# DallinClark/RealTimeRaytracer

Hardware: AMD Instinct MI355X
Metric: Mrays/sec at 1920x1080 1spp (all rays: primary + shadow) (higher is better)
Workload: dtype f32

## Files before the change

realtimeraytracer_amd/csrc/kernels/rtr_device.h:

```cpp
#pragma once
#include <hip/hip_runtime.h>
#include <stdint.h>
#include "../../../include/rtr_types.h"
#include "../../../include/rtr_math.h"

namespace rtrdev {

struct DeviceTexture { const uint8_t* pixels; uint32_t width, height, channels, _pad; };

constexpr uint32_t kLightTriRecord = 4;

struct DeviceScene {
    const uint4* nodes;
    const RtrBvhGrid* grid;
    const uint4* nodes4;
    uint32_t numNodes4;
    const float4* tris;
    const RtrVertex* vertices;
    const uint32_t* indices;
    const RtrObjectInfo* objects;
    const RtrAreaLightInfo* lights;
    const float4* lightTris;
    const uint32_t* lightTriFirst;
    const float* xforms;
    const float* nmats;
    const float* ltc1;
    const float* ltc2;
    float skyLinear[3];
    uint32_t numLights;
    uint32_t numLightTris;
    const DeviceTexture* textures;
    DeviceTexture hdri;
};

struct Counters {
// ... 251 lines not shown
    if (LIMIT > 0 && over) { best.custom = RTR_STACK_OVERFLOW; best.prim = RTR_MISS; best.t = tmax; best.u = 0.f; best.v = 0.f; best.leaf = 0; return false; }
    return found;
}

#define RTR_PI_F 3.14159265359f
__device__ __forceinline__ float chiGGX(float v) { return v > 0.0f ? 1.0f : 0.0f; }
__device__ __forceinline__ float GGX_Distribution(rtr_v3 n, rtr_v3 h, float alpha) {
    const float NoH = rtr_dot(n, h);
    const float alpha2 = alpha * alpha;
    const float NoH2 = NoH * NoH;
    const float den = rtr_max(rtr_fma(NoH2, alpha2, 1.0f - NoH2), 0.001f);
    return (chiGGX(NoH) * alpha2) / (RTR_PI_F * den * den);
}
__device__ __forceinline__ float GGX_PartialGeometryTerm(rtr_v3 v, rtr_v3 n, rtr_v3 h, float alpha) {
    float VoH2 = rtr_clamp(rtr_dot(v, h), 0.001f, 1.0f);
    const float chi = chiGGX(VoH2 / rtr_clamp(rtr_dot(v, n), 0.001f, 1.0f));
    VoH2 = VoH2 * VoH2;
    const float tan2 = (1.0f - VoH2) / VoH2;
    return (chi * 2.0f) / (1.0f + rtr_sqrt(rtr_fma(alpha * alpha, tan2, 1.0f)));
}
__device__ __forceinline__ rtr_v3 Fresnel_Schlick(float cosT, rtr_v3 F0) {
    const float p = rtr_pow(1.0f - cosT, 5.0f);
    return rtr_mk(rtr_fma(1.0f - F0.x, p, F0.x), rtr_fma(1.0f - F0.y, p, F0.y), rtr_fma(1.0f - F0.z, p, F0.z));
}

#define RTR_LUT_SIZE 64.0f
#define RTR_LUT_SCALE ((RTR_LUT_SIZE - 1.0f) / RTR_LUT_SIZE)
#define RTR_LUT_BIAS (0.5f / RTR_LUT_SIZE)

__device__ __forceinline__ float4 sample_lut(const float* __restrict__ lut, float u, float v) {
    float x = rtr_fma(u, RTR_LUT_SIZE, -0.5f), y = rtr_fma(v, RTR_LUT_SIZE, -0.5f);
    if (!(x >= -1.0e6f && x <= 1.0e6f)) x = 0.0f;
    if (!(y >= -1.0e6f && y <= 1.0e6f)) y = 0.0f;
    const float x0f = __builtin_floorf(x), y0f = __builtin_floorf(y);
// ... 81 lines not shown
    return (size_t)(ra.directRows ? gy : lrow) * ra.width + px;
}

__device__ __forceinline__ rtr_v3 primary_dir(const RenderArgs& ra, uint32_t px, uint32_t py, uint32_t i) {
    const float jx = rtr_random(px + i), jy = rtr_random(px + i * 322u);
    const float offx = ((float)px + jx) - 0.5f, offy = ((float)py + jy) - 0.5f;
    const rtr_v3 pw = rtr_madd(rtr_madd(rtr_ld3(ra.cam.topLeftViewportCorner), rtr_ld3(ra.cam.horizontalViewportDelta), offx),
                               rtr_ld3(ra.cam.verticalViewportDelta), offy);
    return rtr_normalize(rtr_sub(pw, rtr_ld3(ra.cam.position)));
}

struct Accum { rtr_v3 analytic, shadowed, unshadowed, avgNormal, avgPosition; };

struct Surface {
    rtr_v3 hitPoint, hitNormal, viewDir, color, mDiffuse, mSpecular;
    float roughness, metallic, om;
    float4 t1, t2;
};

template <bool SHADE, bool STATS>
__device__ __forceinline__ bool fetch_surface(const DeviceScene& sc, const RenderArgs& ra, const HitRec& h, rtr_v3 rayDir,
                                              bool wantAnalytic, Accum& o, Surface& sf, LocalStats& st) {
    if (h.custom == RTR_MISS) {
        if (SHADE) {
            rtr_v3 sky = rtr_ld3(sc.skyLinear);
            if (sc.hdri.pixels) {
                const rtr_v3 dir = rtr_normalize(rayDir);
                const float hu = rtr_atan2(dir.z, dir.x) / (2.0f * 3.14159265f) + 0.5f;
                float hv = rtr_acos(rtr_clamp(dir.y, -1.0f, 1.0f)) / 3.14159265f;
                hv = 1.0f - hv;
                const float4 tx = sample_tex<STATS>(sc.hdri, hu, hv, st);
                sky = rtr_mk(rtr_to_linear(tx.x), rtr_to_linear(tx.y), rtr_to_linear(tx.z));
            }
// ... 24 lines not shown
    const rtr_v3 localPos = rtr_madd(rtr_madd(rtr_scale(p0, b0), p1, b1), p2, b2);
    const rtr_v3 hitPoint = rtr_xform_point34(sc.xforms + 12u * h.custom, localPos);
    const rtr_v3 nsum = rtr_madd(rtr_madd(rtr_scale(n0, b0), n1, b1), n2, b2);
    const float* nm = sc.nmats + 12u * h.custom;
    rtr_v3 hitNormal;
    if (rtr_dot(nsum, nsum) > 0.0f) {
        hitNormal = rtr_normalize(rtr_mul33(nm, rtr_normalize(nsum)));
    } else {
        const rtr_v3 g = rtr_cross(rtr_sub(p1, p0), rtr_sub(p2, p0));
        rtr_v3 n = rtr_normalize(rtr_mul33(nm, rtr_normalize(g)));
        if (rtr_dot(n, rayDir) > 0.0f) n = rtr_neg(n);
        hitNormal = n;
    }
    float metallic = oi->metallic;
    float rough = oi->specular;
    rtr_v3 color = rtr_mk(0, 0, 0);
    if (SHADE) {
        rtr_v3 col = rtr_ld3(oi->color);
        if (oi->usesColorMap | oi->usesSpecularMap | oi->usesMetallicMap) {
            const float4 ta = va[2], tb = vb[2], tc = vc[2];
            const float uu = rtr_fma(tc.x, b2, rtr_fma(tb.x, b1, ta.x * b0));
            const float vv = rtr_fma(tc.y, b2, rtr_fma(tb.y, b1, ta.y * b0));
            if (oi->usesColorMap != 0u) { const float4 t = sample_tex<STATS>(sc.textures[oi->colorIndex], uu, vv, st); col = rtr_mk(t.x, t.y, t.z); }
            if (oi->usesSpecularMap != 0u) rough = sample_tex<STATS>(sc.textures[oi->specularIndex], uu, vv, st).x;
            if (oi->usesMetallicMap != 0u) metallic = sample_tex<STATS>(sc.textures[oi->metallicIndex], uu, vv, st).x;
        }
        color = rtr_mk(rtr_to_linear(col.x), rtr_to_linear(col.y), rtr_to_linear(col.z));
    }
    const float roughness = 1.0f - rough;

    const rtr_v3 viewDir = rtr_normalize(rtr_sub(camPos, hitPoint));
    const float om = 1.0f - metallic;
    rtr_v3 mDiffuse = rtr_mk(0, 0, 0), mSpecular = rtr_mk(0, 0, 0);
    float4 t1 = make_float4(1, 0, 0, 1), t2 = make_float4(0, 0, 0, 0);
    if (SHADE) {
        o.avgNormal = rtr_add(o.avgNormal, hitNormal);
        o.avgPosition = rtr_add(o.avgPosition, hitPoint);
        mDiffuse = rtr_scale(color, om);
        mSpecular = rtr_mk(rtr_fma(color.x, metallic, 0.04f * om), rtr_fma(color.y, metallic, 0.04f * om),
                           rtr_fma(color.z, metallic, 0.04f * om));
        if (wantAnalytic) {
            const float dotNV = rtr_clamp(rtr_dot(hitNormal, viewDir), 0.0f, 1.0f);
            const float lu = rtr_fma(roughness, RTR_LUT_SCALE, RTR_LUT_BIAS);
            const float lv = rtr_fma(rtr_sqrt(1.0f - dotNV), RTR_LUT_SCALE, RTR_LUT_BIAS);
            t1 = sample_lut(sc.ltc1, lu, lv);
            t2 = sample_lut(sc.ltc2, lu, lv);
        }
    }
    sf.hitPoint = hitPoint; sf.hitNormal = hitNormal; sf.viewDir = viewDir; sf.color = color;
    sf.mDiffuse = mDiffuse; sf.mSpecular = mSpecular; sf.roughness = roughness; sf.metallic = metallic; sf.om = om;
    sf.t1 = t1; sf.t2 = t2;
    return true;
}

__device__ __forceinline__ rtr_v3 surface_diffuse(float om, rtr_v3 color) {
    return rtr_mk((om * color.x) / RTR_PI_F, (om * color.y) / RTR_PI_F, (om * color.z) / RTR_PI_F);
}
__device__ __forceinline__ rtr_v3 area_sample_contrib(rtr_v3 hitNormal, rtr_v3 viewDir, float roughness, rtr_v3 mSpecular, rtr_v3 currDiffuse,
                                                      rtr_v3 lcol, float lintensity, float pdf, rtr_v3 sampledLightDir, float lightDistance) {
    const rtr_v3 halfVector = rtr_normalize(rtr_add(viewDir, sampledLightDir));
    const float cosTheta = rtr_clamp(rtr_dot(viewDir, halfVector), 0.0f, 1.0f);
    const float Dg = GGX_Distribution(hitNormal, halfVector, roughness);
    const float G = GGX_PartialGeometryTerm(viewDir, hitNormal, halfVector, roughness) *
                    GGX_PartialGeometryTerm(sampledLightDir, hitNormal, halfVector, roughness);
    const rtr_v3 F = Fresnel_Schlick(cosTheta, mSpecular);
    const float NdotV = rtr_max(rtr_dot(hitNormal, viewDir), 0.1f);
    const float NdotL = rtr_max(rtr_dot(hitNormal, sampledLightDir), 0.1f);
    const float den = 4.0f * NdotV * NdotL;
    const rtr_v3 currSpecular = rtr_mk(((Dg * F.x) * G) / den, ((Dg * F.y) * G) / den, ((Dg * F.z) * G) / den);
    const float attenuation = 1.0f / (lightDistance * lightDistance);
    const rtr_v3 BRDF = rtr_add(currSpecular, currDiffuse);
    const rtr_v3 Lr = rtr_mk((((lcol.x * lintensity) * NdotL) * attenuation) * 10.0f, (((lcol.y * lintensity) * NdotL) * attenuation) * 10.0f,
// ... 34 lines not shown
    return light_sample_at(P, light_sample_pair(s + light_sample_seed0(px, py, frame)));
}
struct DrawnSamples {
    uint32_t px, py, frame;
    __device__ __forceinline__ SamplePair pair(uint32_t s) const { return light_sample_pair(s + light_sample_seed0(px, py, frame)); }
};

constexpr uint32_t kDirectionalSlot = 0xffffffffu;
#ifndef RTR_INTO_EXPR
#define RTR_INTO_EXPR (rtr_dot(hitNormal, lightVec) < 0.0f)
#endif
template <class Policy, bool STATS, class Samples>
__device__ __forceinline__ void light_loops_from(const DeviceScene& sc, const RenderArgs& ra, const Samples& smp,
                                                 const Surface& sf, uint32_t want, Accum& o, Policy& pol, LocalStats& st) {
    const bool wantAnalytic = (want & 1u) != 0u, wantUnshadowed = (want & 2u) != 0u;
    const rtr_v3 hitPoint = sf.hitPoint, hitNormal = sf.hitNormal, viewDir = sf.viewDir, color = sf.color;
    const rtr_v3 mDiffuse = sf.mDiffuse, mSpecular = sf.mSpecular;
    const float roughness = sf.roughness, om = sf.om;
    const float4 t1 = sf.t1, t2 = sf.t2;
    const rtr_v3 shadowOrigin = rtr_madd(hitPoint, hitNormal, 0.01f);
    const rtr_v3 currDiffuse = surface_diffuse(om, color);

    for (uint32_t li = 0; li < ra.info.numAreaLights; ++li) {
        const RtrAreaLightInfo* L = sc.lights + li;
        if (STATS) st.lightFetch++;
        const rtr_v3 lcol = rtr_ld3(L->color);
        const float lintensity = L->intensity;
        const uint32_t lnt = L->numTriangles;
        const bool twoSided = L->isTwoSided != 0u;
        for (uint32_t ti = 0; ti < lnt; ++ti) {
            if (STATS) st.lightTriFetch++;
            const float4* rec = sc.lightTris + (size_t)(sc.lightTriFirst[li] + ti) * kLightTriRecord;
            const float4 r0 = rec[0], r1 = rec[1], r2 = rec[2], r3 = rec[3];
            rtr_v3 P[3];
            P[0] = rtr_mk(r0.x, r0.y, r0.z); P[1] = rtr_mk(r1.x, r1.y, r1.z); P[2] = rtr_mk(r2.x, r2.y, r2.z);
            const float pdf = r1.w;
// ... 152 lines not shown
```

realtimeraytracer_amd/csrc/kernels/rtr_kernels.h:

```cpp
#pragma once
#include <hip/hip_runtime.h>
#include "rtr_device.h"

namespace rtrdev {

#ifndef RTR_SHADOW_FAR_FIRST
#define RTR_SHADOW_FAR_FIRST 1
#endif
#if RTR_SHADOW_FAR_FIRST
#define RTR_ANYHIT_KERNEL_REVISION "r05.3"
#else
#define RTR_ANYHIT_KERNEL_REVISION "r05.3-nearest-first"
#endif

constexpr uint32_t kQueueRegions = 8;
constexpr uint32_t kQueueLenWord = 0;
constexpr uint32_t kPrimaryRedoWord = 2;
constexpr uint32_t kOccludedWord = 3;
constexpr uint32_t kBatchCursorWord = 16;
static_assert(kOccludedWord < kBatchCursorWord && kPrimaryRedoWord < kOccludedWord, "the small counters sit below the first batch cursor");
constexpr uint32_t kQueueLists = kQueueRegions * kQueueRegions;
constexpr uint32_t kQueueListLens = kBatchCursorWord + 16 * kQueueLists;
constexpr uint32_t kPrimaryCursors = kQueueListLens + kQueueLists;
constexpr uint32_t kQueueCtrlWords = kPrimaryCursors + 16 * kQueueRegions;
// ... 71 lines not shown
    uint2* lists;
    uint32_t listStride;
    const int32_t* startLeaves;
    uint32_t numTris;
};
struct RayMaskArgs {
    const uint8_t* rayMasks = nullptr;
    uint32_t cullMask = 0xffu;
    uint32_t masked = 0;
};
hipError_t launch_occlusion_walk(const DeviceScene& sc, const OcclusionArgs& oa, const Tunables& tun, bool alpha, Counters* stats, hipStream_t stream, uint32_t numCus,
                                 const RayMaskArgs& rm = RayMaskArgs());

hipError_t launch_light_tris(const RtrAreaLightInfo* lights, const RtrVertex* vertices, const uint32_t* indices, const uint32_t* first,
                             uint32_t numLights, float4* out, hipStream_t stream);
hipError_t launch_deinterleave(const uint32_t* gathered, uint32_t* dst, uint32_t width, uint32_t height,
                               uint32_t bandRows, uint32_t shardCount, uint32_t localRows, hipStream_t stream);

}
```

realtimeraytracer_amd/csrc/kernels/rtr_kernels.hip:

```cpp
#include "rtr_kernels.h"

#include <algorithm>
#include <cstdlib>
#include <cstring>

namespace rtrdev {

constexpr int kBlock = 256;

template <bool STATS, int STACK>
struct InlinePolicy {
    static constexpr bool kShade = true;
    __device__ __forceinline__ void slots_at(uint32_t) {}
    const DeviceScene& sc; int32_t* stack; LocalStats& st;
    __device__ __forceinline__ bool occluded(rtr_v3 o, rtr_v3 d, float tmax, rtr_v3, bool) {
        HitRec h;
        return trace<true, STATS, kBlock>(sc, stack, o, d, 0.001f, tmax, h, st);
    }
};

__device__ __forceinline__ uint32_t wave_sum_u32(uint32_t v) {
#pragma unroll
    for (int o = 32; o > 0; o >>= 1) v += __shfl_xor(v, o);
    return v;
// ... 393 lines not shown
            }
        }
    }
}

constexpr size_t kBinnedMinRays = (size_t)10 << 20;
constexpr uint32_t kBinnedMinNodes = 1u << 16;
#ifndef RTR_GEN_OCT_BLOCK
#define RTR_GEN_OCT_BLOCK 512
#endif
constexpr uint32_t kGenOctBlock = RTR_GEN_OCT_BLOCK;
constexpr uint32_t kParkSurface = 6, kParkWords = kParkSurface + 2u * kParkedPairs;
#ifndef RTR_GEN_OCT_WAVES
#define RTR_GEN_OCT_WAVES 7
#endif
#if RTR_GEN_OCT_WAVES > 0
#define RTR_GEN_OCT_ATTR __attribute__((amdgpu_waves_per_eu(RTR_GEN_OCT_WAVES, 8)))
#else
#define RTR_GEN_OCT_ATTR
#endif
__global__ __launch_bounds__(kGenOctBlock) RTR_GEN_OCT_ATTR void k_shadow_gen_oct(DeviceScene sc, FrameBatch fb, const float4* hitTuvp, const uint32_t* hitCustom,
                                                              RayQueue queue, uint32_t* ctrl, uint32_t planeStride, uint2* lists,
                                                              uint32_t listStride, uint32_t kBatch, uint32_t nt) {
    constexpr uint32_t kWaves = kGenOctBlock / 64;
    __shared__ uint32_t s_tot[kWaves][8], s_run[kWaves][8];
    __shared__ uint32_t s_park[kParkWords * kGenOctBlock];
    uint32_t q;
    const uint32_t frame = batch_frame(blockIdx.x * kGenOctBlock + threadIdx.x, planeStride, q);
    const RenderArgs& ra = fb.ra[frame < fb.n ? frame : 0u];
    const size_t plane0 = (size_t)frame * ra.spp;
    const uint32_t wave = threadIdx.x >> 6;
    uint32_t px = 0, lrow = 0, py = 0;
    const bool live = frame < fb.n && pixel_of(ra, q, px, lrow, py);
    LocalStats st;
    Accum acc = zero_accum();
    const bool single = ra.spp == 1u;
    const lds_column park = (lds_column)&s_park[threadIdx.x];
    const ParkedSamples<kGenOctBlock> smp{park + kParkSurface * kGenOctBlock, light_sample_seed0(px, py, ra.info.frame), ra.numShadowRays <= kParkedPairs};
    CountOctPolicy cp{0ull, 0ull};
    if (live) {
        smp.draw(ra.numShadowRays);
        for (uint32_t i = 0; i < ra.spp; ++i) {
            const size_t k = (plane0 + i) * planeStride + q;
            const float4 r = hitTuvp[k];
            HitRec h; h.t = r.x; h.u = r.y; h.v = r.z; h.prim = __float_as_uint(r.w); h.custom = hitCustom[k];
            Surface sf;
            bool surf = fetch_surface<false, false>(sc, ra, h, primary_dir(ra, px, py, i), false, acc, sf, st);
#if RTR_EXP_DOUBLE_FETCH_GEN
            if (surf) {
                HitRec h2 = h; h2.u = h.u + sf.hitPoint.x * (float)(ra.spp - 1u) * 1.0e-30f; h2.v = h.v + sf.hitNormal.y * (float)(ra.spp - 1u) * 1.0e-30f;
                h2.prim = h.prim + (__float_as_uint(sf.hitPoint.z) == 0x7fc12345u ? 1u : 0u);
                Surface sf2;
                if (fetch_surface<false, false>(sc, ra, h2, primary_dir(ra, px, py, i), false, acc, sf2, st)) sf = sf2;
            }
#endif
            if (surf) {
                if (single) {
// ... 39 lines not shown
        uint32_t at = 0, pos = 0;
        if (threadIdx.x == 0 && total) at = atomicAdd(ctrl, total);
        if (cnt) pos = atomicAdd(ctrl + kQueueListLens + threadIdx.x, cnt);
        const uint32_t first = (uint32_t)__builtin_amdgcn_readfirstlane((int)at) + before;
        if (x == 0) {
            uint32_t c = first;
            for (uint32_t w = 0; w < kWaves; ++w) { s_run[w][o] = c; c += s_tot[w][o]; }
        }
        for (uint32_t j = 0; j < cnt; ++j) {
            const uint32_t f = (b0 + j * kQueueRegions) * kB;
            lists[(size_t)threadIdx.x * listStride + pos + j] = make_uint2(first + f, len - f < kB ? len - f : kB);
        }
    }
    __syncthreads();
    if (mine == 0) return;
    for (uint32_t i = 0; i < ra.spp; ++i) {
        const size_t k = (plane0 + i) * planeStride + q;
        EmitOctPolicy pol{queue, (EmitOctPolicy::lds_word)&s_run[wave][0], (uint32_t)k, nt};
        if (single) {
            Surface sf0 = {};
            sf0.hitPoint = rtr_mk(__uint_as_float(park[0u * kGenOctBlock]), __uint_as_float(park[1u * kGenOctBlock]), __uint_as_float(park[2u * kGenOctBlock]));
            sf0.hitNormal = rtr_mk(__uint_as_float(park[3u * kGenOctBlock]), __uint_as_float(park[4u * kGenOctBlock]), __uint_as_float(park[5u * kGenOctBlock]));
            queue_store_origin(queue, k, sf0.hitPoint, sf0.hitNormal);
            light_loops_from<EmitOctPolicy, false>(sc, ra, smp, sf0, 0u, acc, pol, st);
        } else {
            const float4 r = hitTuvp[k];
            HitRec h; h.t = r.x; h.u = r.y; h.v = r.z; h.prim = __float_as_uint(r.w); h.custom = hitCustom[k];
            Surface sf;
            if (fetch_surface<false, false>(sc, ra, h, primary_dir(ra, px, py, i), false, acc, sf, st)) {
                queue_store_origin(queue, k, sf.hitPoint, sf.hitNormal);
                light_loops_from<EmitOctPolicy, false>(sc, ra, smp, sf, 0u, acc, pol, st);
            }
        }
    }
// ... 882 lines not shown
        if (valid) {
            const float4 r = hitTuvp[k];
            HitRec h; h.t = r.x; h.u = r.y; h.v = r.z; h.prim = __float_as_uint(r.w); h.custom = hitCustom[k];
            has = fetch_surface<true, false>(sc, ra, h, primary_dir(ra, px, py, i), false, acc, sf, st);
#if RTR_EXP_DOUBLE_FETCH
            if (has) {
                HitRec h2 = h; h2.u = h.u + (float)(ra.spp - 1u) * 1.0e-30f; h2.v = h.v + (float)(ra.spp - 1u) * 1.0e-30f;
                Surface sf2; Accum acc2 = zero_accum();
                const bool has2 = fetch_surface<true, false>(sc, ra, h2, primary_dir(ra, px, py, i), false, acc2, sf2, st);
                if (has2 && sf2.roughness == 12345.0f && sf2.hitPoint.x == 4321.0f && sf2.color.y == 777.0f && sf2.viewDir.z == 55.0f && sf2.hitNormal.y == 99.0f) sf = sf2;
            }
#endif
        }
        wave_lds_sync();
        if (has) {
            const rtr_v3 cd = surface_diffuse(sf.om, sf.color);
            s_surf[wave][0][lane] = make_float4(sf.hitPoint.x, sf.hitPoint.y, sf.hitPoint.z, sf.roughness);
            s_surf[wave][1][lane] = make_float4(sf.hitNormal.x, sf.hitNormal.y, sf.hitNormal.z, cd.x);
            s_surf[wave][2][lane] = make_float4(sf.viewDir.x, sf.viewDir.y, sf.viewDir.z, cd.y);
            s_surf[wave][3][lane] = make_float4(sf.mSpecular.x, sf.mSpecular.y, sf.mSpecular.z, cd.z);
        }
        const rtr_v3 hitPoint = sf.hitPoint, hitNormal = sf.hitNormal;
        uint32_t qdone = 0;
        rtr_v3 shadowedSample = rtr_mk(0, 0, 0);
        uint32_t e0 = 0, total = 0;
        do {
            uint32_t count = 0, e = 0, e1 = e0;
            uint32_t vmask = 0, imask = 0;
            bool full = false;
            const uint32_t occ = has ? vis_mask32(vis, (uint32_t)k + qdone * slotStride, slotStride, ra.maxRaysPerSample - qdone) : 0xffffffffu;
            uint32_t nq = 0;
// ... 101 lines not shown
        const uint32_t band = y / bandRows, r = y % bandRows;
        const uint32_t shard = band % shardCount, lb = band / shardCount;
        dst[p] = gathered[((size_t)shard * localRows + (size_t)lb * bandRows + r) * width + x];
    }
}

__global__ __launch_bounds__(64) void k_light_tris(const RtrAreaLightInfo* __restrict__ lights, const RtrVertex* __restrict__ vertices,
                                                   const uint32_t* __restrict__ indices, const uint32_t* __restrict__ first,
                                                   uint32_t numLights, float4* __restrict__ out) {
    const uint32_t l = blockIdx.x * 64u + threadIdx.x;
    if (l >= numLights) return;
    const RtrAreaLightInfo* L = lights + l;
    for (uint32_t ti = 0; ti < L->numTriangles; ++ti) light_tri_record(L, vertices, indices, ti, out + (size_t)(first[l] + ti) * kLightTriRecord);
}

__global__ __launch_bounds__(kBlock) void k_fill_planes(uint4* __restrict__ vis, uint32_t word, uint32_t planeVec, uint32_t pitchVec,
                                                        uint32_t* __restrict__ ctrl, uint32_t ctrlWords, uint32_t* __restrict__ overflowCount) {
    if (blockIdx.x == 0 && blockIdx.y == 0) {
        for (uint32_t i = threadIdx.x; i < ctrlWords; i += kBlock) ctrl[i] = 0u;
        if (threadIdx.x == 0) overflowCount[0] = 0u;
    }
    const uint4 v = make_uint4(word, word, word, word);
    uint4* plane = vis + (size_t)blockIdx.y * pitchVec;
    for (uint32_t i = blockIdx.x * kBlock + threadIdx.x; i < planeVec; i += gridDim.x * kBlock) plane[i] = v;
}

namespace {
struct TunableField { const char* name; uint32_t Tunables::* field; uint32_t lo, hi; };
const TunableField kTunables[] = {
    {"primary_packet", &Tunables::primary_packet, 0u, 1u}, {"primary_wide", &Tunables::primary_wide, 0u, 1u}, {"primary_persist", &Tunables::primary_persist, 0u, 2u}, {"primary_persist_min_rays", &Tunables::primary_persist_min_rays, 0u, 0xffffffffu},
// ... 96 lines not shown
    }
    if (ev) hipEventRecord(ev[1], s);
    const uint32_t kBatchEnv = tun.trace_batch;
    const uint32_t kBatch = kBatchEnv >= 64u ? kBatchEnv : ((size_t)nb * blocks * kBlock * ra.spp * ra.maxRaysPerSample >= kBatchLongQueue ? kBatchLong : kBatchDefault);
    const uint32_t kWide = tun.trace_bvh4;
    const uint32_t genBlocks = (nb * blocks * kBlock + kGenBlock - 1) / kGenBlock, genOctBlocks = (nb * blocks * kBlock + kGenOctBlock - 1) / kGenOctBlock;
    const uint32_t binMode = tun.trace_binned;
    const size_t maxRaysQ = (size_t)nb * blocks * kBlock * ra.spp * ra.maxRaysPerSample;
    const bool wide = kWide && sc.nodes4;
    const bool binned = wide && ws.batchLists && (size_t)ra.spp * ra.maxRaysPerSample <= 65535u &&
                        (size_t)ws.capRays / kBatch / kQueueRegions + genOctBlocks <= ws.listStride &&
                        (binMode == 1u || (binMode == 2u && maxRaysQ >= kBinnedMinRays && sc.numNodes4 >= kBinnedMinNodes));
    const uint32_t kNtQueue = tun.queue_nt;
    RayQueue rq = ws.rayQueue;
    rq.ownLeaf = (wide && tun.trace_own_leaf) ? 1u : 0u;
    if (binned) hipLaunchKernelGGL(k_shadow_gen_oct, dim3(genOctBlocks), dim3(kGenOctBlock), 0, s, sc, fb, ws.hitTuvp, ws.hitCustom, rq, ws.queueCount, blocks * kBlock, ws.batchLists, ws.listStride, kBatch, kNtQueue >> 1);
    else hipLaunchKernelGGL(k_shadow_gen, dim3(genBlocks), dim3(kGenBlock), 0, s, sc, fb, ws.hitTuvp, ws.hitCustom, rq, ws.queueCount, blocks * kBlock);
    if (ev) hipEventRecord(ev[2], s);
    const size_t maxRays = (size_t)nb * blocks * kBlock * ra.spp * ra.maxRaysPerSample;
    const uint32_t kWgsPerCu = tun.trace_wgs_per_cu;
    uint32_t tblocks = numCus * (kWgsPerCu ? kWgsPerCu : (maxRays >= kBinnedMinRays ? 8u : 6u));
    const uint32_t needed = (uint32_t)((maxRays + kBlock - 1) / kBlock);
    if (tblocks > needed) tblocks = needed;
    if (tblocks == 0) tblocks = 1;
    const uint32_t kRefill = tun.trace_refill, kInnerMin = tun.trace_inner_min;
    (void)sizeof(STACK);
    const uint32_t kOct = tun.trace_octant_forms | ((kNtQueue & 1u) << 1);
    const uint32_t kTop = tun.trace_top_nodes < kTopNodes ? tun.trace_top_nodes : kTopNodes;
    const uint32_t top = kTop < sc.numNodes4 ? kTop : sc.numNodes4;
    uint32_t tblocks4 = tblocks * (uint32_t)kBlock / (uint32_t)kTraceBlock;
    if (tblocks4 == 0) tblocks4 = 1;
// ... 64 lines not shown
        if (hinted) { if (stats) RTR_OCC_WALK(true, true, true); else RTR_OCC_WALK(false, true, true); }
        else { if (stats) RTR_OCC_WALK(true, false, true); else RTR_OCC_WALK(false, false, true); }
    } else if (hinted) { if (stats) RTR_OCC_WALK(true, true, false); else RTR_OCC_WALK(false, true, false); }
    else { if (stats) RTR_OCC_WALK(true, false, false); else RTR_OCC_WALK(false, false, false); }
#undef RTR_OCC_WALK
    return hipGetLastError();
}

hipError_t launch_light_tris(const RtrAreaLightInfo* lights, const RtrVertex* vertices, const uint32_t* indices, const uint32_t* first,
                             uint32_t numLights, float4* out, hipStream_t stream) {
    if (numLights == 0) return hipSuccess;
    hipLaunchKernelGGL(k_light_tris, dim3((numLights + 63u) / 64u), dim3(64), 0, stream, lights, vertices, indices, first, numLights, out);
    return hipGetLastError();
}

hipError_t launch_deinterleave(const uint32_t* gathered, uint32_t* dst, uint32_t width, uint32_t height,
                               uint32_t bandRows, uint32_t shardCount, uint32_t localRows, hipStream_t stream) {
    const size_t total = (size_t)width * height;
    uint32_t blocks = (uint32_t)((total + kBlock - 1) / kBlock);
    if (blocks > 2048u) blocks = 2048u;
    if (blocks == 0) blocks = 1;
    hipLaunchKernelGGL(k_deinterleave, dim3(blocks), dim3(kBlock), 0, stream, gathered, dst, width, height, bandRows, shardCount, localRows);
    return hipGetLastError();
}

}
```

realtimeraytracer_amd/csrc/kernels/rtr_query.hip:

```cpp
#include "rtr_query_device.h"
#include "../../../include/rtr.h"
#include "../../../include/rtr_pick.h"
#include "../../../include/rtr_mis.h"

namespace rtrdev {

#ifndef RTR_PRIMARY_BLOCK
#define RTR_PRIMARY_BLOCK 64
#endif
constexpr int kQueryBlock = RTR_PRIMARY_BLOCK;
static_assert(kQueryBlock % 64 == 0 && kQueryBlock >= 64 && kQueryBlock <= 1024, "RTR_PRIMARY_BLOCK: a multiple of 64");
constexpr int kQueryTailBlock = 256;
constexpr int kQueryTailBlocks = 64;
static_assert((size_t)64 * kQueryTailBlocks * kQueryTailBlock == kSpillInts, "the tail kernel's stacks fill the spill area");
constexpr uint8_t kOccludedRedo = 0xffu;

__device__ __forceinline__ void query_store_hit(float4* __restrict__ hits, uint32_t k, const HitRec& h) {
    hits[2 * (size_t)k] = make_float4(h.t, h.u, h.v, __uint_as_float(h.custom));
    hits[2 * (size_t)k + 1] = make_float4(__uint_as_float(h.prim), 0.0f, 0.0f, 0.0f);
}

__device__ __forceinline__ uint32_t query_cull(const RayMaskArgs& rm) { return rm.masked & kCullAll; }
static_assert(kCullBackFacing == RTR_QUERY_CULL_BACK_FACING && kCullFrontFacing == RTR_QUERY_CULL_FRONT_FACING && kCullOpaque == RTR_QUERY_CULL_OPAQUE &&
              kCullNoOpaque == RTR_QUERY_CULL_NO_OPAQUE && (kCullAll & 1u) == 0u, "the kernels' cull bits are the interface's");
// ... 528 lines not shown
    const LightArgs& la = pa.la;
    const uint32_t k = blockIdx.x * kShadeBlock + threadIdx.x;
    if (k >= la.n) return;
    HitRec h;
    rtr_v3 dir;
    RenderArgs ra{};
    const uint32_t kind = light_hit(sc, la, k, h, dir, ra);
    const bool wantUnshadowed = (la.outputs & RTR_LIGHT_UNSHADOWED) != 0u;
    const rtr_v3 zero = rtr_mk(0, 0, 0);
    const uint32_t P = pa.picks, R = P + 1u;
    Accum acc;
    acc.analytic = acc.shadowed = acc.unshadowed = acc.avgNormal = acc.avgPosition = zero;
    Surface sf;
    LocalStats st;
    if (kind != RTR_SURFACE_INVALID && fetch_surface<true, false>(sc, ra, h, dir, false, acc, sf, st)) {
        const rtr_v3 currDiffuse = surface_diffuse(sf.om, sf.color);
        const uint8_t* occ = la.occluded + (size_t)k * R;
        rtr_v3 sumShadowed = zero, sumUnshadowed = zero;
        for (uint32_t p = 0; p < P; ++p) {
            const size_t at = (size_t)k * P + p;
            const uint32_t j = pa.slotsIn[at];
            PickedSample ps;
            if (j >= pa.areaSlots || !picked_sample(sc, pa, ra, sf.hitPoint, j, ps)) continue;
            const bool occluded = occ[p] != 0;
            if (wantUnshadowed || !occluded) {
                const float w = pa.weights ? pa.weights[at] : pa.defaultWeight;
                const rtr_v3 contrib = area_sample_contrib(sf.hitNormal, sf.viewDir, sf.roughness, sf.mSpecular, currDiffuse, ps.lcol, ps.lintensity, ps.pdf, ps.dir, ps.dist);
                sumShadowed = rtr_madd(sumShadowed, contrib, occluded ? 0.0f : w);
                sumUnshadowed = rtr_madd(sumUnshadowed, contrib, w);
            }
        }
// ... 80 lines not shown
```

realtimeraytracer_amd/csrc/rtr_api.cpp:

```cpp
#include "../../include/rtr.h"
#include "../../include/rtr_math.h"
#include "bvh_build.h"
#include "kernels/rtr_kernels.h"
#include "kernels/rtr_post.h"
#include "kernels/rtr_bvh.h"
#include "kernels/rtr_mirrored.h"
#include "kernels/rtr_tree_sah.h"
#include "kernels/rtr_query.h"
#include "kernels/rtr_bounce_launch.h"
#include "rtr_bounce_host.h"
#include "kernels/rtr_paths_launch.h"
#include "rtr_paths_host.h"
#include "rtr_pick_host.h"
#include "kernels/rtr_mis_launch.h"
#include "rtr_mis_host.h"

#include <hip/hip_runtime.h>

#include <algorithm>
#include <chrono>
#include <cstdarg>
#include <cstdio>
#include <cstring>
#include <string>
// ... 129 lines not shown
    mutable int costParentState = 0;
    DevBuf<uint32_t> orderScratch;
    bool asyncReady = false;
    bool rebuildReady = false;
    bool rebuildIfReady = false;
    rtr_scene_stats stats{};
};
}

struct rtr_scene {
    rtr_ctx* ctx = nullptr;
    SceneTree tree;
    DevBuf<RtrVertex> vertices;
    DevBuf<uint32_t> indices;
    DevBuf<RtrObjectInfo> objects;
    DevBuf<RtrAreaLightInfo> lights;
    DevBuf<float4> lightTris;
    DevBuf<uint32_t> lightTriFirst;
    DevBuf<uint32_t> triCount;
    uint32_t numInstances = 0;
    std::vector<uint8_t> hostMasks;
    DevBuf<uint32_t> maskBits;
    std::vector<uint32_t> hostTriCount;
    mutable DevBuf<uint32_t> leafBase;
    DevBuf<float> xforms, nmats, ltc1, ltc2;
    std::vector<DevBuf<uint8_t>> texPixels;
    DevBuf<uint8_t> hdriPixels;
    DevBuf<rtrdev::DeviceTexture> texTable;
    std::vector<RtrAreaLightInfo> hostLights;
    std::vector<RtrInstance> hostInstances;
// ... 359 lines not shown
        if (s->numLights) HIP_TRY(hipMemcpy(s->hostLights.data(), s->lights.p, s->numLights * sizeof(RtrAreaLightInfo), hipMemcpyDeviceToHost));
        s->instancesStale = false;
    }
    s->mirrorsStale = false;
    return RTR_OK;
}

static int make_light_tris(rtr_scene* s) {
    if (s->numLights == 0) return RTR_OK;
    hipError_t e = rtrdev::launch_light_tris(s->lights.p, s->vertices.p, s->indices.p, s->lightTriFirst.p, s->numLights, s->lightTris.p, s->ctx->stream);
    if (e != hipSuccess) return fail(RTR_ERR_HIP, "light-triangle records: %s", hipGetErrorString(e));
    HIP_TRY(hipStreamSynchronize(s->ctx->stream));
    return RTR_OK;
}

static int make_wide_nodes(SceneTree& t, hipStream_t st) {
    const uint32_t n = (uint32_t)t.hostNodes.size();
    if (!t.nodes4.p) { HIP_TRY(t.nodes4.alloc((size_t)n * 4)); HIP_TRY(t.nodes4tmp.alloc((size_t)n * 4)); HIP_TRY(t.wideRemap.alloc(n)); HIP_TRY(t.wideSums.alloc(rtrdev::bvh_wide_scratch_words())); }
    if (!t.hostWideShape.empty() && !t.wideShape.p) HIP_TRY(t.wideShape.upload(t.hostWideShape.data(), t.hostWideShape.size(), st));
    hipError_t e = rtrdev::bvh_make_wide(t.nodes.p, n, t.refitReady ? t.parent.p : nullptr, t.grid.p, t.hostWideShape.size() == n ? t.wideShape.p : nullptr, t.nodes4tmp.p, t.wideSums.p, st);
    if (e != hipSuccess) return fail(RTR_ERR_HIP, "4-wide node build: %s", hipGetErrorString(e));
    std::vector<uint32_t> codes((size_t)n * 4), remap(n, 0xffffffffu), order;
    HIP_TRY(hipMemcpy2DAsync(codes.data(), 16, reinterpret_cast<const char*>(t.nodes4tmp.p) + 48, 64, 16, n, hipMemcpyDeviceToHost, st));
    HIP_TRY(hipStreamSynchronize(st));
    order.reserve(n);
    order.push_back(0); remap[0] = 0;
    for (size_t head = 0; head < order.size(); ++head)
        for (int k = 0; k < 4; ++k) {
            const int32_t c = (int32_t)codes[(size_t)order[head] * 4 + k];
            if (c >= 0 && (uint32_t)c < n && remap[c] == 0xffffffffu) { remap[c] = (uint32_t)order.size(); order.push_back((uint32_t)c); }
// ... 174 lines not shown
    if (d->numMeshes) s->hostMeshes.assign(d->meshes, d->meshes + d->numMeshes);
    if (d->numObjects) s->hostObjects.assign(d->objects, d->objects + d->numObjects);
    if (deviceBuild) {
        rc = build_on_device(s, d, totalPrims);
        if (rc != RTR_OK) { delete s; ctx_release_child(ctx); return rc; }
    } else {
        fill_stats(tree.stats, bvh, stackEntries, numTris);
        tree.hostNodes.swap(bvh.nodes);
        tree.hostTris.swap(bvh.tris);
        tree.hostWideShape.swap(bvh.wideShape);
        tree.numPrims = (uint32_t)tree.hostTris.size(); tree.numNodeSlots = (uint32_t)tree.hostNodes.size();
    }

    rc = make_wide_nodes(tree, st);
    if (rc == RTR_OK) rc = make_light_tris(s);
    if (rc != RTR_OK) { delete s; ctx_release_child(ctx); return rc; }
    DeviceScene& dv = s->dev;
    point_at_tree(dv, tree);
    dv.vertices = s->vertices.p; dv.indices = s->indices.p;
    dv.objects = s->objects.p; dv.lights = s->lights.p;
    dv.lightTris = s->lightTris.p; dv.lightTriFirst = s->lightTriFirst.p;
    dv.xforms = s->xforms.p; dv.nmats = s->nmats.p;
    dv.ltc1 = s->hasLtc ? s->ltc1.p : nullptr; dv.ltc2 = s->hasLtc ? s->ltc2.p : nullptr;
    for (int k = 0; k < 3; ++k) dv.skyLinear[k] = rtr_to_linear(d->skyColor[k]);
    dv.numLights = d->numLights;
    dv.numLightTris = 0;
    for (uint32_t l = 0; l < d->numLights; ++l) dv.numLightTris += d->lights[l].numTriangles;
    dv.textures = s->texTable.p;
    dv.hdri = hdri;
    *out = s;
    return RTR_OK;
}

int rtr_scene_create(rtr_ctx* ctx, const rtr_scene_desc* d, rtr_scene** out) { return scene_create_impl(ctx, d, nullptr, out); }

// ... 1939 lines not shown
    if (!s) return fail(RTR_ERR_INVALID_ARGUMENT, "%s: null scene", who);
    uint32_t total = 0;
    std::vector<uint32_t> first(s->numLights);
    for (uint32_t l = 0; l < s->numLights; ++l) { first[l] = total; total += s->hostLights[l].numTriangles; }
    if (outCount) *outCount = total;
    if (capacityTris < total || (total && !outRecords))
        return fail(RTR_ERR_INVALID_ARGUMENT, "%s: capacity %u light triangles, %u are needed", who, outRecords ? capacityTris : 0u, total);
    HIP_TRY(hipSetDevice(s->ctx->device));
    hipStream_t st = s->ctx->stream;
    if (total) HIP_TRY(hipMemcpyAsync(outRecords, s->lightTris.p, (size_t)total * rtrdev::kLightTriRecord * sizeof(float4), hipMemcpyDeviceToHost, st));
    HIP_TRY(hipStreamSynchronize(st));
    if (outFirst) for (uint32_t l = 0; l < s->numLights; ++l) outFirst[l] = first[l];
    return RTR_OK;
}

}
```

Before: 16520.

## Precompute per-object material terms and specialize shadow-gen kernel for single spp

Adds a per-object table of linearized color, diffuse/specular terms and roughness, built once at scene creation, so untextured hits load four float4s instead of recomputing sRGB conversions and material terms per hit. The shadow generation kernel becomes a template on SINGLE, with spp fixed at compile time and a higher waves-per-EU hint for the 1spp case, which should cut registers and branches. It also drops the chi term in the GGX geometry function. That term's argument is a ratio of two values clamped to at least 0.001, so it is always 1 and removing it changes nothing. The Surface struct gains a diffuse field, which may raise register pressure elsewhere. The table is indexed by h.custom minus numLights, which assumes light objects come first.

```diff
diff --git a/realtimeraytracer_amd/csrc/kernels/rtr_device.h b/realtimeraytracer_amd/csrc/kernels/rtr_device.h
--- a/realtimeraytracer_amd/csrc/kernels/rtr_device.h
+++ b/realtimeraytracer_amd/csrc/kernels/rtr_device.h
@@ -9,6 +9,7 @@
 struct DeviceTexture { const uint8_t* pixels; uint32_t width, height, channels, _pad; };
 
 constexpr uint32_t kLightTriRecord = 4;
+constexpr uint32_t kObjectTermsRecord = 4;
 
 struct DeviceScene {
     const uint4* nodes;
@@ -19,6 +20,7 @@
     const RtrVertex* vertices;
     const uint32_t* indices;
     const RtrObjectInfo* objects;
+    const float4* objectTerms;
     const RtrAreaLightInfo* lights;
     const float4* lightTris;
     const uint32_t* lightTriFirst;
@@ -300,10 +302,9 @@
 }
 __device__ __forceinline__ float GGX_PartialGeometryTerm(rtr_v3 v, rtr_v3 n, rtr_v3 h, float alpha) {
     float VoH2 = rtr_clamp(rtr_dot(v, h), 0.001f, 1.0f);
-    const float chi = chiGGX(VoH2 / rtr_clamp(rtr_dot(v, n), 0.001f, 1.0f));
     VoH2 = VoH2 * VoH2;
     const float tan2 = (1.0f - VoH2) / VoH2;
-    return (chi * 2.0f) / (1.0f + rtr_sqrt(rtr_fma(alpha * alpha, tan2, 1.0f)));
+    return 2.0f / (1.0f + rtr_sqrt(rtr_fma(alpha * alpha, tan2, 1.0f)));
 }
 __device__ __forceinline__ rtr_v3 Fresnel_Schlick(float cosT, rtr_v3 F0) {
     const float p = rtr_pow(1.0f - cosT, 5.0f);
@@ -415,9 +416,34 @@
 
 struct Surface {
     rtr_v3 hitPoint, hitNormal, viewDir, color, mDiffuse, mSpecular;
+    rtr_v3 diffuse;
     float roughness, metallic, om;
     float4 t1, t2;
 };
+
+__device__ __forceinline__ rtr_v3 surface_diffuse(float om, rtr_v3 color) {
+    return rtr_mk((om * color.x) / RTR_PI_F, (om * color.y) / RTR_PI_F, (om * color.z) / RTR_PI_F);
+}
+__device__ __forceinline__ void material_terms(rtr_v3 color, float metallic, float om, rtr_v3& mDiffuse, rtr_v3& mSpecular, rtr_v3& diffuse) {
+    mDiffuse = rtr_scale(color, om);
+    mSpecular = rtr_mk(rtr_fma(color.x, metallic, 0.04f * om), rtr_fma(color.y, metallic, 0.04f * om),
+                       rtr_fma(color.z, metallic, 0.04f * om));
+    diffuse = surface_diffuse(om, color);
+}
+__device__ __forceinline__ void object_terms_record(const RtrObjectInfo* oi, float4* rec) {
+    const rtr_v3 col = rtr_ld3(oi->color);
+    const rtr_v3 color = rtr_mk(rtr_to_linear(col.x), rtr_to_linear(col.y), rtr_to_linear(col.z));
+    const float metallic = oi->metallic;
+    const float roughness = 1.0f - oi->specular;
+    const float om = 1.0f - metallic;
+    rtr_v3 mDiffuse, mSpecular, diffuse;
+    material_terms(color, metallic, om, mDiffuse, mSpecular, diffuse);
+    const uint32_t plain = (oi->usesColorMap | oi->usesSpecularMap | oi->usesMetallicMap) == 0u ? 1u : 0u;
+    rec[0] = make_float4(color.x, color.y, color.z, roughness);
+    rec[1] = make_float4(mDiffuse.x, mDiffuse.y, mDiffuse.z, metallic);
+    rec[2] = make_float4(mSpecular.x, mSpecular.y, mSpecular.z, om);
+    rec[3] = make_float4(diffuse.x, diffuse.y, diffuse.z, __uint_as_float(plain));
+}
 
 template <bool SHADE, bool STATS>
 __device__ __forceinline__ bool fetch_surface(const DeviceScene& sc, const RenderArgs& ra, const HitRec& h, rtr_v3 rayDir,
@@ -472,31 +498,41 @@
     }
     float metallic = oi->metallic;
     float rough = oi->specular;
-    rtr_v3 color = rtr_mk(0, 0, 0);
+    rtr_v3 color = rtr_mk(0, 0, 0), mDiffuse = rtr_mk(0, 0, 0), mSpecular = rtr_mk(0, 0, 0), diffuse = rtr_mk(0, 0, 0);
+    float roughness = 0.0f, om = 0.0f;
+    bool tabled = false;
     if (SHADE) {
-        rtr_v3 col = rtr_ld3(oi->color);
-        if (oi->usesColorMap | oi->usesSpecularMap | oi->usesMetallicMap) {
+        const float4* ot = sc.objectTerms + (size_t)kObjectTermsRecord * (h.custom - sc.numLights);
+        const float4 m3 = ot[3];
+        tabled = __float_as_uint(m3.w) != 0u;
+        if (tabled) {
+            const float4 m0 = ot[0], m1 = ot[1], m2 = ot[2];
+            color = rtr_mk(m0.x, m0.y, m0.z); roughness = m0.w;
+            mDiffuse = rtr_mk(m1.x, m1.y, m1.z); metallic = m1.w;
+            mSpecular = rtr_mk(m2.x, m2.y, m2.z); om = m2.w;
+            diffuse = rtr_mk(m3.x, m3.y, m3.z);
+        } else {
+            rtr_v3 col = rtr_ld3(oi->color);
             const float4 ta = va[2], tb = vb[2], tc = vc[2];
             const float uu = rtr_fma(tc.x, b2, rtr_fma(tb.x, b1, ta.x * b0));
             const float vv = rtr_fma(tc.y, b2, rtr_fma(tb.y, b1, ta.y * b0));
             if (oi->usesColorMap != 0u) { const float4 t = sample_tex<STATS>(sc.textures[oi->colorIndex], uu, vv, st); col = rtr_mk(t.x, t.y, t.z); }
             if (oi->usesSpecularMap != 0u) rough = sample_tex<STATS>(sc.textures[oi->specularIndex], uu, vv, st).x;
             if (oi->usesMetallicMap != 0u) metallic = sample_tex<STATS>(sc.textures[oi->metallicIndex], uu, vv, st).x;
-        }
-        color = rtr_mk(rtr_to_linear(col.x), rtr_to_linear(col.y), rtr_to_linear(col.z));
-    }
-    const float roughness = 1.0f - rough;
+            color = rtr_mk(rtr_to_linear(col.x), rtr_to_linear(col.y), rtr_to_linear(col.z));
+        }
+    }
+    if (!tabled) {
+        roughness = 1.0f - rough;
+        om = 1.0f - metallic;
+        if (SHADE) material_terms(color, metallic, om, mDiffuse, mSpecular, diffuse);
+    }
 
     const rtr_v3 viewDir = rtr_normalize(rtr_sub(camPos, hitPoint));
-    const float om = 1.0f - metallic;
-    rtr_v3 mDiffuse = rtr_mk(0, 0, 0), mSpecular = rtr_mk(0, 0, 0);
     float4 t1 = make_float4(1, 0, 0, 1), t2 = make_float4(0, 0, 0, 0);
     if (SHADE) {
         o.avgNormal = rtr_add(o.avgNormal, hitNormal);
         o.avgPosition = rtr_add(o.avgPosition, hitPoint);
-        mDiffuse = rtr_scale(color, om);
-        mSpecular = rtr_mk(rtr_fma(color.x, metallic, 0.04f * om), rtr_fma(color.y, metallic, 0.04f * om),
-                           rtr_fma(color.z, metallic, 0.04f * om));
         if (wantAnalytic) {
             const float dotNV = rtr_clamp(rtr_dot(hitNormal, viewDir), 0.0f, 1.0f);
             const float lu = rtr_fma(roughness, RTR_LUT_SCALE, RTR_LUT_BIAS);
@@ -506,14 +542,11 @@
         }
     }
     sf.hitPoint = hitPoint; sf.hitNormal = hitNormal; sf.viewDir = viewDir; sf.color = color;
-    sf.mDiffuse = mDiffuse; sf.mSpecular = mSpecular; sf.roughness = roughness; sf.metallic = metallic; sf.om = om;
+    sf.mDiffuse = mDiffuse; sf.mSpecular = mSpecular; sf.diffuse = diffuse; sf.roughness = roughness; sf.metallic = metallic; sf.om = om;
     sf.t1 = t1; sf.t2 = t2;
     return true;
 }
 
-__device__ __forceinline__ rtr_v3 surface_diffuse(float om, rtr_v3 color) {
-    return rtr_mk((om * color.x) / RTR_PI_F, (om * color.y) / RTR_PI_F, (om * color.z) / RTR_PI_F);
-}
 __device__ __forceinline__ rtr_v3 area_sample_contrib(rtr_v3 hitNormal, rtr_v3 viewDir, float roughness, rtr_v3 mSpecular, rtr_v3 currDiffuse,
                                                       rtr_v3 lcol, float lintensity, float pdf, rtr_v3 sampledLightDir, float lightDistance) {
     const rtr_v3 halfVector = rtr_normalize(rtr_add(viewDir, sampledLightDir));
@@ -578,12 +611,12 @@
 __device__ __forceinline__ void light_loops_from(const DeviceScene& sc, const RenderArgs& ra, const Samples& smp,
                                                  const Surface& sf, uint32_t want, Accum& o, Policy& pol, LocalStats& st) {
     const bool wantAnalytic = (want & 1u) != 0u, wantUnshadowed = (want & 2u) != 0u;
-    const rtr_v3 hitPoint = sf.hitPoint, hitNormal = sf.hitNormal, viewDir = sf.viewDir, color = sf.color;
+    const rtr_v3 hitPoint = sf.hitPoint, hitNormal = sf.hitNormal, viewDir = sf.viewDir;
     const rtr_v3 mDiffuse = sf.mDiffuse, mSpecular = sf.mSpecular;
-    const float roughness = sf.roughness, om = sf.om;
+    const float roughness = sf.roughness;
     const float4 t1 = sf.t1, t2 = sf.t2;
     const rtr_v3 shadowOrigin = rtr_madd(hitPoint, hitNormal, 0.01f);
-    const rtr_v3 currDiffuse = surface_diffuse(om, color);
+    const rtr_v3 currDiffuse = sf.diffuse;
 
     for (uint32_t li = 0; li < ra.info.numAreaLights; ++li) {
         const RtrAreaLightInfo* L = sc.lights + li;
diff --git a/realtimeraytracer_amd/csrc/kernels/rtr_kernels.h b/realtimeraytracer_amd/csrc/kernels/rtr_kernels.h
--- a/realtimeraytracer_amd/csrc/kernels/rtr_kernels.h
+++ b/realtimeraytracer_amd/csrc/kernels/rtr_kernels.h
@@ -109,6 +109,8 @@
 
 hipError_t launch_light_tris(const RtrAreaLightInfo* lights, const RtrVertex* vertices, const uint32_t* indices, const uint32_t* first,
                              uint32_t numLights, float4* out, hipStream_t stream);
+hipError_t launch_object_terms(const RtrObjectInfo* objects, uint32_t numObjects, float4* out, hipStream_t stream);
+hipError_t gen_oct_attributes(bool single, hipFuncAttributes* out);
 hipError_t launch_deinterleave(const uint32_t* gathered, uint32_t* dst, uint32_t width, uint32_t height,
                                uint32_t bandRows, uint32_t shardCount, uint32_t localRows, hipStream_t stream);
 
diff --git a/realtimeraytracer_amd/csrc/kernels/rtr_kernels.hip b/realtimeraytracer_amd/csrc/kernels/rtr_kernels.hip
--- a/realtimeraytracer_amd/csrc/kernels/rtr_kernels.hip
+++ b/realtimeraytracer_amd/csrc/kernels/rtr_kernels.hip
@@ -431,33 +431,31 @@
 #ifndef RTR_GEN_OCT_WAVES
 #define RTR_GEN_OCT_WAVES 7
 #endif
-#if RTR_GEN_OCT_WAVES > 0
-#define RTR_GEN_OCT_ATTR __attribute__((amdgpu_waves_per_eu(RTR_GEN_OCT_WAVES, 8)))
-#else
-#define RTR_GEN_OCT_ATTR
-#endif
-__global__ __launch_bounds__(kGenOctBlock) RTR_GEN_OCT_ATTR void k_shadow_gen_oct(DeviceScene sc, FrameBatch fb, const float4* hitTuvp, const uint32_t* hitCustom,
-                                                              RayQueue queue, uint32_t* ctrl, uint32_t planeStride, uint2* lists,
-                                                              uint32_t listStride, uint32_t kBatch, uint32_t nt) {
+template <bool SINGLE>
+__global__ __launch_bounds__(kGenOctBlock) __attribute__((amdgpu_waves_per_eu(SINGLE ? 8 : RTR_GEN_OCT_WAVES, 8)))
+void k_shadow_gen_oct(DeviceScene sc, FrameBatch fb, const float4* hitTuvp, const uint32_t* hitCustom,
+                      RayQueue queue, uint32_t* ctrl, uint32_t planeStride, uint2* lists,
+                      uint32_t listStride, uint32_t kBatch, uint32_t nt) {
     constexpr uint32_t kWaves = kGenOctBlock / 64;
     __shared__ uint32_t s_tot[kWaves][8], s_run[kWaves][8];
     __shared__ uint32_t s_park[kParkWords * kGenOctBlock];
     uint32_t q;
     const uint32_t frame = batch_frame(blockIdx.x * kGenOctBlock + threadIdx.x, planeStride, q);
     const RenderArgs& ra = fb.ra[frame < fb.n ? frame : 0u];
-    const size_t plane0 = (size_t)frame * ra.spp;
+    const uint32_t spp = SINGLE ? 1u : ra.spp;
+    const size_t plane0 = (size_t)frame * spp;
     const uint32_t wave = threadIdx.x >> 6;
     uint32_t px = 0, lrow = 0, py = 0;
     const bool live = frame < fb.n && pixel_of(ra, q, px, lrow, py);
     LocalStats st;
     Accum acc = zero_accum();
-    const bool single = ra.spp == 1u;
+    constexpr bool single = SINGLE;
     const lds_column park = (lds_column)&s_park[threadIdx.x];
     const ParkedSamples<kGenOctBlock> smp{park + kParkSurface * kGenOctBlock, light_sample_seed0(px, py, ra.info.frame), ra.numShadowRays <= kParkedPairs};
     CountOctPolicy cp{0ull, 0ull};
     if (live) {
         smp.draw(ra.numShadowRays);
-        for (uint32_t i = 0; i < ra.spp; ++i) {
+        for (uint32_t i = 0; i < spp; ++i) {
             const size_t k = (plane0 + i) * planeStride + q;
             const float4 r = hitTuvp[k];
             HitRec h; h.t = r.x; h.u = r.y; h.v = r.z; h.prim = __float_as_uint(r.w); h.custom = hitCustom[k];
@@ -527,10 +525,10 @@
     }
     __syncthreads();
     if (mine == 0) return;
-    for (uint32_t i = 0; i < ra.spp; ++i) {
+    for (uint32_t i = 0; i < spp; ++i) {
         const size_t k = (plane0 + i) * planeStride + q;
         EmitOctPolicy pol{queue, (EmitOctPolicy::lds_word)&s_run[wave][0], (uint32_t)k, nt};
-        if (single) {
+        if constexpr (single) {
             Surface sf0 = {};
             sf0.hitPoint = rtr_mk(__uint_as_float(park[0u * kGenOctBlock]), __uint_as_float(park[1u * kGenOctBlock]), __uint_as_float(park[2u * kGenOctBlock]));
             sf0.hitNormal = rtr_mk(__uint_as_float(park[3u * kGenOctBlock]), __uint_as_float(park[4u * kGenOctBlock]), __uint_as_float(park[5u * kGenOctBlock]));
@@ -1443,7 +1441,7 @@
         }
         wave_lds_sync();
         if (has) {
-            const rtr_v3 cd = surface_diffuse(sf.om, sf.color);
+            const rtr_v3 cd = sf.diffuse;
             s_surf[wave][0][lane] = make_float4(sf.hitPoint.x, sf.hitPoint.y, sf.hitPoint.z, sf.roughness);
             s_surf[wave][1][lane] = make_float4(sf.hitNormal.x, sf.hitNormal.y, sf.hitNormal.z, cd.x);
             s_surf[wave][2][lane] = make_float4(sf.viewDir.x, sf.viewDir.y, sf.viewDir.z, cd.y);
@@ -1575,6 +1573,12 @@
     for (uint32_t ti = 0; ti < L->numTriangles; ++ti) light_tri_record(L, vertices, indices, ti, out + (size_t)(first[l] + ti) * kLightTriRecord);
 }
 
+__global__ __launch_bounds__(64) void k_object_terms(const RtrObjectInfo* __restrict__ objects, uint32_t numObjects, float4* __restrict__ out) {
+    const uint32_t o = blockIdx.x * 64u + threadIdx.x;
+    if (o >= numObjects) return;
+    object_terms_record(objects + o, out + (size_t)o * kObjectTermsRecord);
+}
+
 __global__ __launch_bounds__(kBlock) void k_fill_planes(uint4* __restrict__ vis, uint32_t word, uint32_t planeVec, uint32_t pitchVec,
                                                         uint32_t* __restrict__ ctrl, uint32_t ctrlWords, uint32_t* __restrict__ overflowCount) {
     if (blockIdx.x == 0 && blockIdx.y == 0) {
@@ -1701,7 +1705,8 @@
     const uint32_t kNtQueue = tun.queue_nt;
     RayQueue rq = ws.rayQueue;
     rq.ownLeaf = (wide && tun.trace_own_leaf) ? 1u : 0u;
-    if (binned) hipLaunchKernelGGL(k_shadow_gen_oct, dim3(genOctBlocks), dim3(kGenOctBlock), 0, s, sc, fb, ws.hitTuvp, ws.hitCustom, rq, ws.queueCount, blocks * kBlock, ws.batchLists, ws.listStride, kBatch, kNtQueue >> 1);
+    if (binned && ra.spp == 1u) hipLaunchKernelGGL(k_shadow_gen_oct<true>, dim3(genOctBlocks), dim3(kGenOctBlock), 0, s, sc, fb, ws.hitTuvp, ws.hitCustom, rq, ws.queueCount, blocks * kBlock, ws.batchLists, ws.listStride, kBatch, kNtQueue >> 1);
+    else if (binned) hipLaunchKernelGGL(k_shadow_gen_oct<false>, dim3(genOctBlocks), dim3(kGenOctBlock), 0, s, sc, fb, ws.hitTuvp, ws.hitCustom, rq, ws.queueCount, blocks * kBlock, ws.batchLists, ws.listStride, kBatch, kNtQueue >> 1);
     else hipLaunchKernelGGL(k_shadow_gen, dim3(genBlocks), dim3(kGenBlock), 0, s, sc, fb, ws.hitTuvp, ws.hitCustom, rq, ws.queueCount, blocks * kBlock);
     if (ev) hipEventRecord(ev[2], s);
     const size_t maxRays = (size_t)nb * blocks * kBlock * ra.spp * ra.maxRaysPerSample;
@@ -1796,6 +1801,17 @@
     return hipGetLastError();
 }
 
+hipError_t launch_object_terms(const RtrObjectInfo* objects, uint32_t numObjects, float4* out, hipStream_t stream) {
+    if (numObjects == 0) return hipSuccess;
+    hipLaunchKernelGGL(k_object_terms, dim3((numObjects + 63u) / 64u), dim3(64), 0, stream, objects, numObjects, out);
+    return hipGetLastError();
+}
+
+hipError_t gen_oct_attributes(bool single, hipFuncAttributes* out) {
+    return single ? hipFuncGetAttributes(out, reinterpret_cast<const void*>(&k_shadow_gen_oct<true>))
+                  : hipFuncGetAttributes(out, reinterpret_cast<const void*>(&k_shadow_gen_oct<false>));
+}
+
 hipError_t launch_deinterleave(const uint32_t* gathered, uint32_t* dst, uint32_t width, uint32_t height,
                                uint32_t bandRows, uint32_t shardCount, uint32_t localRows, hipStream_t stream) {
     const size_t total = (size_t)width * height;
diff --git a/realtimeraytracer_amd/csrc/kernels/rtr_query.hip b/realtimeraytracer_amd/csrc/kernels/rtr_query.hip
--- a/realtimeraytracer_amd/csrc/kernels/rtr_query.hip
+++ b/realtimeraytracer_amd/csrc/kernels/rtr_query.hip
@@ -566,7 +566,7 @@
     Surface sf;
     LocalStats st;
     if (kind != RTR_SURFACE_INVALID && fetch_surface<true, false>(sc, ra, h, dir, false, acc, sf, st)) {
-        const rtr_v3 currDiffuse = surface_diffuse(sf.om, sf.color);
+        const rtr_v3 currDiffuse = sf.diffuse;
         const uint8_t* occ = la.occluded + (size_t)k * R;
         rtr_v3 sumShadowed = zero, sumUnshadowed = zero;
         for (uint32_t p = 0; p < P; ++p) {
diff --git a/realtimeraytracer_amd/csrc/rtr_api.cpp b/realtimeraytracer_amd/csrc/rtr_api.cpp
--- a/realtimeraytracer_amd/csrc/rtr_api.cpp
+++ b/realtimeraytracer_amd/csrc/rtr_api.cpp
@@ -167,6 +167,7 @@
     DevBuf<RtrVertex> vertices;
     DevBuf<uint32_t> indices;
     DevBuf<RtrObjectInfo> objects;
+    DevBuf<float4> objectTerms;
     DevBuf<RtrAreaLightInfo> lights;
     DevBuf<float4> lightTris;
     DevBuf<uint32_t> lightTriFirst;
@@ -556,6 +557,15 @@
     return RTR_OK;
 }
 
+static int make_object_terms(rtr_scene* s) {
+    if (s->numObjects == 0) return RTR_OK;
+    HIP_TRY(s->objectTerms.alloc((size_t)s->numObjects * rtrdev::kObjectTermsRecord));
+    hipError_t e = rtrdev::launch_object_terms(s->objects.p, s->numObjects, s->objectTerms.p, s->ctx->stream);
+    if (e != hipSuccess) return fail(RTR_ERR_HIP, "object terms: %s", hipGetErrorString(e));
+    HIP_TRY(hipStreamSynchronize(s->ctx->stream));
+    return RTR_OK;
+}
+
 static int make_wide_nodes(SceneTree& t, hipStream_t st) {
     const uint32_t n = (uint32_t)t.hostNodes.size();
     if (!t.nodes4.p) { HIP_TRY(t.nodes4.alloc((size_t)n * 4)); HIP_TRY(t.nodes4tmp.alloc((size_t)n * 4)); HIP_TRY(t.wideRemap.alloc(n)); HIP_TRY(t.wideSums.alloc(rtrdev::bvh_wide_scratch_words())); }
@@ -760,11 +770,12 @@
 
     rc = make_wide_nodes(tree, st);
     if (rc == RTR_OK) rc = make_light_tris(s);
+    if (rc == RTR_OK) rc = make_object_terms(s);
     if (rc != RTR_OK) { delete s; ctx_release_child(ctx); return rc; }
     DeviceScene& dv = s->dev;
     point_at_tree(dv, tree);
     dv.vertices = s->vertices.p; dv.indices = s->indices.p;
-    dv.objects = s->objects.p; dv.lights = s->lights.p;
+    dv.objects = s->objects.p; dv.objectTerms = s->objectTerms.p; dv.lights = s->lights.p;
     dv.lightTris = s->lightTris.p; dv.lightTriFirst = s->lightTriFirst.p;
     dv.xforms = s->xforms.p; dv.nmats = s->nmats.p;
     dv.ltc1 = s->hasLtc ? s->ltc1.p : nullptr; dv.ltc2 = s->hasLtc ? s->ltc2.p : nullptr;
@@ -2734,4 +2745,14 @@
     return RTR_OK;
 }
 
-}
+#ifdef RTR_TEST_HOOKS
+int rtr_test_gen_oct_attributes(int single, uint32_t out[4]) {
+    if (!out) return fail(RTR_ERR_INVALID_ARGUMENT, "rtr_test_gen_oct_attributes: null output");
+    hipFuncAttributes a{};
+    HIP_TRY(rtrdev::gen_oct_attributes(single != 0, &a));
+    out[0] = (uint32_t)a.numRegs; out[1] = (uint32_t)a.localSizeBytes; out[2] = (uint32_t)a.sharedSizeBytes; out[3] = (uint32_t)a.maxThreadsPerBlock;
+    return RTR_OK;
+}
+#endif
+
+}
```

Result: faster. 16710, median of 6 (+1.1%).
